# MakiseChris666/MVXNet-Makise

Measured on AMD Instinct MI355X. Metric: KITTI frames/sec (voxelize+VFE+fusion+3Dconv fwd+bwd), higher is better.
Workload: dtype f32 (bf16x6: three bf16 pieces = the f32 operand exactly, six MFMAs per product, f32 accumulate); 1 GPU; S2 ring frames (64-beam model, KITTI-like occupancy), 120000 raw pts -> 20000 pts after crop, grid 10x352x400, T=35, 4 frames/GPU/step: crop+cropToSight+lidar2Img, voxelize, fusion sampling+MLP, VFE, reindex+CML fwd+bwd, all-reduce, AdamW; convmath=bf16x6; mode=hot, frames_per_gpu=4, parallelism=dp1

## Files before the change

mvxnet-makise_amd/csrc/conv3d_split.hip:

```cpp
#include "common.h"
#include "conv_geom.h"
#include "split_common.h"
#include "rowgemm_common.h"

namespace {

constexpr int TH2 = 16;

__global__ void pack_weights_split(const float *__restrict__ w, unsigned short *__restrict__ wsp, int Co, int Ci, int dgrad, int np, int fmt) {
    const int K = dgrad ? Co : Ci, N = dgrad ? Ci : Co;
    const int nch = K / BK;
    const long long total = 27ll * K * N;
    for (long long e = blockIdx.x * (long long)blockDim.x + threadIdx.x; e < total; e += (long long)gridDim.x * blockDim.x) {
        const int k = (int)(e % BK);
        long long r = e / BK;
        const int n = (int)(r % N); r /= N;
        const int ch = (int)(r % nch); r /= nch;
        const int tap = (int)(r % 9);
        const int kd = (int)(r / 9);
        const int a = tap / 3, b = tap % 3;
        const int kk = ch * BK + k;
        const int co = dgrad ? kk : n, ci = dgrad ? n : kk;
        const int kh = dgrad ? 2 - a : a, kw = dgrad ? 2 - b : b;
        float x = w[((((long long)co * Ci + ci) * 3 + kd) * 3 + kh) * 3 + kw];
        const long long row = (((long long)kd * 9 + tap) * nch + ch) * N + n;
        for (int q = 0; q < np; ++q) {
            if (fmt == 0) {
                const __bf16 pb = (__bf16)x;
                wsp[(row * np + q) * BK + k] = __builtin_bit_cast(unsigned short, pb);
                x -= (float)pb;
            } else {
                if (q == 0) x *= SPLIT_F16_WSCALE;
                const _Float16 pb = (_Float16)x;
                wsp[(row * np + q) * BK + k] = __builtin_bit_cast(unsigned short, pb);
                x -= (float)pb;
            }
        }
    }
}

template <int NP, int BKT, int MT, bool WIN, int FMT>
__global__ __launch_bounds__(256, 2) void conv3d_gather_splitT(const float *__restrict__ in,
                                                               const unsigned short *__restrict__ wsp,
                                                               const float *__restrict__ bias,
                                                               float *__restrict__ out, double *__restrict__ stats,
                                                               Geom g, int relu, const int *__restrict__ in_hflag,
                                                               const unsigned char *__restrict__ out_mask,
                                                               const float *__restrict__ bg_pre, int border_active,
                                                               const int *__restrict__ only_tiles,
                                                               unsigned long long *__restrict__ exec_stages,
                                                               const float *__restrict__ in_amax) {
    float a_scale = 1.f;
    if constexpr (FMT == 1) a_scale = split_scale_of(in_amax);
    constexpr int THT = TH * MT, HHT = THT + 2;
    constexpr int ROWBT = NP * BKT * 2 + 16;
    constexpr int HROW = (HW * ROWBT + 255) / 256 * 256;
    constexpr int PPR = NP * BKT / 8;
    constexpr int PT = BN * PPR;
    constexpr int NWU = (3 * PT + 255) / 256;
    constexpr int PARTS = BKT / 4;
    constexpr int NH = (HHT * HW * PARTS + 255) / 256;
    constexpr int KS = BKT / 16;
    __shared__ __attribute__((aligned(256))) unsigned char s_halo[HHT * HROW];
    __shared__ __attribute__((aligned(16))) unsigned char s_w[3][BN * ROWBT];
    __shared__ float s_red[4][2 * BN];
    const int tiles_x = (g.W + TW - 1) / TW, tiles_y8 = (g.H + TH - 1) / TH;
    const int ntiles8 = tiles_x * tiles_y8;
    const int tx = blockIdx.x % tiles_x, tyb = blockIdx.x / tiles_x;
    const int tx0 = tx * TW, ty0 = tyb * THT;
    const int t_top = (MT * tyb) * tiles_x + tx;
    const bool has_bot = MT == 2 && 2 * tyb + 1 < tiles_y8;
    const int t_bot = has_bot ? t_top + tiles_x : t_top;
    const int d = blockIdx.y, nb = blockIdx.z;
    const int tid = threadIdx.x, lane = tid & 63, wv = tid >> 6, li = lane & 31, lh = lane >> 5;
    const int nchunks = g.Cin / BKT;
    if (only_tiles && !(only_tiles[(size_t)d * ntiles8 + t_top] | only_tiles[(size_t)d * ntiles8 + t_bot])) return;
    const bool on_border = tx0 == 0 || ty0 == 0 || tx0 + TW >= g.W || ty0 + THT >= g.H;
    const bool skip_taps = in_hflag && (border_active & 2) && !on_border;
    unsigned skipped = 0;
    int any_flag = 0;
    bool active = true;
    if (in_hflag) {
        for (int kd = 0; kd < 3; ++kd) {
            const int ds = src_depth(g, d, kd);
            if (ds >= 0) {
                const int fl = in_hflag[(size_t)ds * ntiles8 + t_top] | in_hflag[(size_t)ds * ntiles8 + t_bot];
                any_flag |= fl;
                if (skip_taps && !fl) skipped |= 1u << kd;
            }
        }
        active = (((border_active & 1) && on_border) || any_flag) != 0;
    }
    const bool idle_border = in_hflag && (border_active & 2) && on_border && !any_flag;

    f32x16 acc[MT][2];
#pragma unroll
    for (int m = 0; m < MT; ++m)
#pragma unroll
        for (int n = 0; n < 2; ++n)
#pragma unroll
            for (int r = 0; r < 16; ++r) acc[m][n][r] = 0.f;
    int a_base[MT];
#pragma unroll
    for (int m = 0; m < MT; ++m) a_base[m] = (2 * MT * wv + 2 * m + (li >> 4)) * HROW + (li & 15) * ROWBT + lh * 16;
    const int b_base = li * ROWBT + lh * 16;

    typedef unsigned u32x4 __attribute__((ext_vector_type(4)));
    u32x4 wreg[NWU];
    auto load_w3 = [&](int kd, int a, int cc) __attribute__((always_inline)) {
        const int c32 = (cc * BKT) / BK, half = BKT == 16 ? (cc & 1) : 0;
#pragma unroll
        for (int u = 0; u < NWU; ++u) {
            int c = tid + 256 * u;
            if (3 * PT % 256 && c >= 3 * PT) c = 3 * PT - 1;
            const int t = c / PT, rem = c - t * PT;
            const int n = rem / PPR, piece = rem - n * PPR;
            const int q = piece / (BKT / 8), sub = piece - q * (BKT / 8);
            const unsigned char *row = (const unsigned char *)wsp +
                (((((size_t)kd * 9 + a * 3 + t) * (g.Cin / BK) + c32) * g.Cout + (size_t)nb * BN + n) * NP + q) * (BK * 2);
            wreg[u] = *(const u32x4 *)(row + half * 32 + sub * 16);
        }
    };
    auto store_w3 = [&]() __attribute__((always_inline)) {
#pragma unroll
        for (int u = 0; u < NWU; ++u) {
            const int c = tid + 256 * u;
            if (3 * PT % 256 == 0 || c < 3 * PT) {
                const int t = c / PT, rem = c - t * PT;
                const int n = rem / PPR, piece = rem - n * PPR;
                *(u32x4 *)(s_w[t] + n * ROWBT + piece * 16) = wreg[u];
            }
        }
    };

    int kd_l[3] = {0, 0, 0}, ds_l[3] = {0, 0, 0}, nk = 0;
#pragma unroll
    for (int kd = 0; kd < 3; ++kd) {
        const int ds = src_depth(g, d, kd);
        if (ds >= 0 && !((skipped >> kd) & 1u) && !idle_border) {
            if (nk == 0) { kd_l[0] = kd; ds_l[0] = ds; }
            else if (nk == 1) { kd_l[1] = kd; ds_l[1] = ds; }
            else { kd_l[2] = kd; ds_l[2] = ds; }
            ++nk;
        }
    }
    const int nstages = active ? nk * nchunks : 0;
    if (exec_stages && nstages > 0 && threadIdx.x == 0)
        atomicAdd(exec_stages, (unsigned long long)(nk * (g.Cin / BK)) * (has_bot ? 2 : 1));
    auto stage_of = [&](int st, int &kd, int &ds, int &cc) __attribute__((always_inline)) {
        const int i = st / nchunks;
        cc = st - i * nchunks;
        kd = i == 0 ? kd_l[0] : (i == 1 ? kd_l[1] : kd_l[2]);
        ds = i == 0 ? ds_l[0] : (i == 1 ? ds_l[1] : ds_l[2]);
    };
    int h_off[NH], h_lds[NH];
#pragma unroll
    for (int u = 0; u < NH; ++u) {
        const int c = tid + 256 * u;
        h_off[u] = -1;
        h_lds[u] = -1;
        if (c < HHT * HW * PARTS) {
            const int r = c / PARTS, part = c - r * PARTS;
            const int hy = r / HW, hx = r - hy * HW;
            const int gy = ty0 - 1 + hy, gx = tx0 - 1 + hx;
            h_lds[u] = hy * HROW + hx * ROWBT + part * 8;
            if (gy >= 0 && gy < g.H && gx >= 0 && gx < g.W) h_off[u] = (gy * g.W + gx) * g.Cin + part * 4;
        }
    }
    f32x4 hreg[NH];
    auto load_halo = [&](int st) __attribute__((always_inline)) {
        int kd, ds, cc;
        stage_of(st, kd, ds, cc);
        const float *img = in + (size_t)ds * g.H * g.W * g.Cin + cc * BKT;
#pragma unroll
        for (int u = 0; u < NH; ++u)
            hreg[u] = h_off[u] >= 0 ? *(const f32x4 *)(img + h_off[u]) : f32x4{0.f, 0.f, 0.f, 0.f};
    };
    auto store_halo = [&]() __attribute__((always_inline)) {
#pragma unroll
        for (int u = 0; u < NH; ++u)
            if (h_lds[u] >= 0) {
                uint2 pc[NP];
                if constexpr (FMT == 1) hreg[u] *= a_scale;
                split_n<NP, FMT>(hreg[u][0], hreg[u][1], hreg[u][2], hreg[u][3], pc);
#pragma unroll
                for (int q = 0; q < NP; ++q) *(uint2 *)(s_halo + h_lds[u] + q * BKT * 2) = pc[q];
            }
    };
    auto load_wrow = [&](int st, int a) __attribute__((always_inline)) {
        int kd, ds, cc;
        stage_of(st, kd, ds, cc);
        load_w3(kd, a, cc);
    };
    auto compute_row = [&](int a, unsigned colmask) __attribute__((always_inline)) {
#pragma unroll
        for (int b = 0; b < 3; ++b) {
            if (!((colmask >> b) & 1u)) continue;
#pragma unroll
            for (int s2 = 0; s2 < KS; ++s2) {
                bf16x8 b0[NP], b1[NP];
#pragma unroll
                for (int q = 0; q < NP; ++q) {
                    b0[q] = __builtin_bit_cast(bf16x8, *(const uint4 *)(s_w[b] + b_base + q * BKT * 2 + s2 * 32));
                    b1[q] = __builtin_bit_cast(bf16x8, *(const uint4 *)(s_w[b] + b_base + 32 * ROWBT + q * BKT * 2 + s2 * 32));
                }
#pragma unroll
                for (int m = 0; m < MT; ++m) {
                    const int a_off = a_base[m] + a * HROW + b * ROWBT + s2 * 32;
                    bf16x8 av[NP];
#pragma unroll
                    for (int q = 0; q < NP; ++q) av[q] = __builtin_bit_cast(bf16x8, *(const uint4 *)(s_halo + a_off + q * BKT * 2));
                    split_mac2<NP, FMT>(acc[m][0], acc[m][1], av, b0, b1);
                }
            }
        }
    };
    if constexpr (!WIN) {
        if (nstages > 0) {
            load_wrow(0, 0);
            load_halo(0);
        }
        for (int st = 0; st < nstages; ++st) {
            const int nxt = st + 1 < nstages ? st + 1 : st;
            __syncthreads();
            store_halo();
            store_w3();
            __syncthreads();
            load_wrow(st, 1);
            load_halo(nxt);
            compute_row(0, 7u);
            __syncthreads();
            store_w3();
            __syncthreads();
            load_wrow(st, 2);
            compute_row(1, 7u);
            __syncthreads();
            store_w3();
            __syncthreads();
            load_wrow(nxt, 0);
            compute_row(2, 7u);
        }
    } else {
        auto taps_of = [&](int st) __attribute__((always_inline)) -> unsigned {
            unsigned m4 = 0xfu;
            if (g.s2d > 0) m4 = s2d_tap_mask(g.mode == 0 ? ((st % nchunks) * BKT) / g.s2d : (nb * BN) / g.s2d);
            unsigned m9 = 0u;
    #pragma unroll
            for (int a = 0; a < 3; ++a)
    #pragma unroll
                for (int b = 0; b < 3; ++b) {
                    const int ta = g.mode == 0 ? a : 2 - a, tb = g.mode == 0 ? b : 2 - b;
                    const bool in = a >= g.tap_lo && a < g.tap_hi && b >= g.tap_lo && b < g.tap_hi;
                    const bool on = g.s2d > 0 ? ((m4 >> ((ta & 1) * 2 + (tb & 1))) & 1u) && ta < 2 && tb < 2 : true;
                    if (in && on) m9 |= 1u << (a * 3 + b);
                }
            return m9;
        };
        auto first_row = [&](unsigned m9) __attribute__((always_inline)) { return (m9 & 7u) ? 0 : ((m9 & 0x38u) ? 1 : 2); };
        auto next_row = [&](unsigned m9, int a) __attribute__((always_inline)) {
            for (int r = a + 1; r < 3; ++r)
                if ((m9 >> (3 * r)) & 7u) return r;
            return -1;
        };
        int st = 0;
        unsigned m9 = nstages > 0 ? taps_of(0) : 0x1ffu;
        int a = first_row(m9);
        if (nstages > 0) {
            load_wrow(0, a);
            load_halo(0);
        }
        while (st < nstages) {
            const bool first = a == first_row(m9);
            int a2 = next_row(m9, a), st2 = st;
            unsigned m9n = m9;
            if (a2 < 0) {
                st2 = st + 1;
                m9n = st2 < nstages ? taps_of(st2) : m9;
                a2 = first_row(m9n);
            }
            const int stp = st2 < nstages ? st2 : st;
            __syncthreads();
            if (first) store_halo();
            store_w3();
            __syncthreads();
            load_wrow(stp, a2);
            if (first) load_halo(st + 1 < nstages ? st + 1 : st);
            compute_row(a, (m9 >> (3 * a)) & 7u);
            st = st2; a = a2; m9 = m9n;
        }
    }

    if constexpr (FMT == 1) {
        const float o_scale = split_inverse(split_scale_of(in_amax)) * (1.f / SPLIT_F16_WSCALE);
#pragma unroll
        for (int m = 0; m < MT; ++m) { acc[m][0] *= o_scale; acc[m][1] *= o_scale; }
    }
    const int n0 = nb * BN + li, n1 = n0 + 32;
    const float bias0 = bias ? bias[n0] : 0.f, bias1 = bias ? bias[n1] : 0.f;
    float skip0 = 0.f, skip1 = 0.f;
    if (skipped && active) {
        const float *bg_tap = bg_pre + (size_t)g.Dout * g.F * g.Cout + (size_t)d * 3 * g.Cout;
#pragma unroll
        for (int kd = 0; kd < 3; ++kd)
            if ((skipped >> kd) & 1u) { skip0 += bg_tap[kd * g.Cout + n0]; skip1 += bg_tap[kd * g.Cout + n1]; }
    }
    float bgv0 = (bg_pre ? bg_pre[(size_t)d * g.Cout + n0] : 0.f) + bias0, bgv1 = (bg_pre ? bg_pre[(size_t)d * g.Cout + n1] : 0.f) + bias1;
    if (relu) { bgv0 = fmaxf(bgv0, 0.f); bgv1 = fmaxf(bgv1, 0.f); }
    float s1a = 0.f, s2a = 0.f, s1b = 0.f, s2b = 0.f;
#pragma unroll
    for (int m = 0; m < MT; ++m) {
        const int py = ty0 + 2 * MT * wv + 2 * m;
        if (idle_border) {
            const float *bg_cls = bg_pre + (size_t)4 * g.Dout * g.F * g.Cout + (size_t)d * 9 * g.Cout;
#pragma unroll
            for (int r = 0; r < 16; ++r) {
                const int row = mfma32_row(r) + 4 * lh;
                const int gy = py + (row >> 4), gx = tx0 + (row & 15);
                const int q = 3 * (gy == 0 ? 0 : (gy >= g.H - 1 ? 2 : 1)) + (gx == 0 ? 0 : (gx >= g.W - 1 ? 2 : 1));
                acc[m][0][r] = bg_cls[q * g.Cout + n0];
                acc[m][1][r] = bg_cls[q * g.Cout + n1];
            }
        }
        unsigned site_on = active ? 0xffffu : 0u;
        if (out_mask && active) {
            unsigned char mk[16];
#pragma unroll
            for (int r = 0; r < 16; ++r) {
                const int row = mfma32_row(r) + 4 * lh;
                const int gy = min(py + (row >> 4), g.H - 1), gx = min(tx0 + (row & 15), g.W - 1);
                mk[r] = out_mask[((size_t)d * g.H + gy) * g.W + gx];
            }
            site_on = 0u;
#pragma unroll
            for (int r = 0; r < 16; ++r) site_on |= (mk[r] ? 1u : 0u) << r;
        }
#pragma unroll
        for (int r = 0; r < 16; ++r) {
            const int row = mfma32_row(r) + 4 * lh;
            const int gy = py + (row >> 4), gx = tx0 + (row & 15);
            float v0 = (acc[m][0][r] + skip0) + bias0, v1 = (acc[m][1][r] + skip1) + bias1;
            if (relu) { v0 = fmaxf(v0, 0.f); v1 = fmaxf(v1, 0.f); }
            if (out_mask && !((site_on >> r) & 1u)) { v0 = bgv0; v1 = bgv1; }
            if (gy < g.H && gx < g.W) {
                float *o = out + (((size_t)d * g.H + gy) * g.W + gx) * g.Cout;
                o[n0] = v0;
                o[n1] = v1;
                s1a += v0; s2a += v0 * v0;
                s1b += v1; s2b += v1 * v1;
            }
        }
    }
    if (stats) {
        s1a += __shfl_xor(s1a, 32, 64); s2a += __shfl_xor(s2a, 32, 64);
        s1b += __shfl_xor(s1b, 32, 64); s2b += __shfl_xor(s2b, 32, 64);
        __syncthreads();
        if (lh == 0) {
            s_red[wv][li] = s1a; s_red[wv][32 + li] = s1b;
            s_red[wv][BN + li] = s2a; s_red[wv][BN + 32 + li] = s2b;
        }
        __syncthreads();
        if (tid < 2 * BN) {
            const double t = (double)s_red[0][tid] + (double)s_red[1][tid] + (double)s_red[2][tid] + (double)s_red[3][tid];
            const int which = tid / BN, c = tid % BN;
            const unsigned rep = (blockIdx.x + blockIdx.y * gridDim.x) % MVX_REP;
            double *fstats = stats + (size_t)(d / g.Dout) * MVX_REP * 2 * g.Cout;
            atomicAdd(fstats + ((size_t)rep * 2 + which) * g.Cout + nb * BN + c, t);
        }
    }
}

static long long g_split16_min_units = 768;

extern "C" int mvx_tuning_set(int32_t key, int64_t value) {
    if (key == MVX_TUNE_SPLIT16_MIN_UNITS) { g_split16_min_units = value; return MVX_OK; }
    if (key == MVX_TUNE_GATHER_NARROW_MAX_UNITS) { mvxi_gather_narrow_max_units(value); return MVX_OK; }
    if (key == MVX_TUNE_ROWGEMM_K128) { mvxi_rowgemm_k128_enable(value); return MVX_OK; }
    return MVX_EINVAL;
}

static inline int pieces_of(int flags) { return (flags & MVX_FLAG_SPLIT_F16) ? 2 : (flags & MVX_FLAG_SPLIT3) ? 3 : 2; }
static inline int fmt_of(int flags) { return (flags & MVX_FLAG_SPLIT_F16) ? 1 : 0; }

static void launch_gather_split(hipStream_t st, int flags, int planes, int nblocks, const float *in, const unsigned short *wsp,
                                const float *bias, float *out, double *stats, const Geom &g, int relu, const int *in_hflag,
                                const unsigned char *out_mask, const float *bg_pre, int border_active, const int *only_tiles,
                                unsigned long long *exec_stages) {
    const int tiles_x = (int)mvx_cdiv(g.W, TW);
    const long long units16 = (long long)tiles_x * mvx_cdiv(g.H, TH2) * planes * nblocks;
    const bool big = units16 >= g_split16_min_units;
    const dim3 grid(tiles_x * mvx_cdiv(g.H, big ? TH2 : TH), planes, nblocks);
    const bool win = g.tap_lo != 0 || g.tap_hi != 3 || g.s2d > 0;
    const SplitAmax am = mvxi_take_split_amax();
#define MVX_GO(NP_, BK_, MT_, F_)                                                                                                        \
    do {                                                                                                                             \
        if (win)                                                                                                                     \
            hipLaunchKernelGGL((conv3d_gather_splitT<NP_, BK_, MT_, true, F_>), grid, dim3(256), 0, st, in, wsp, bias, out, stats, g,    \
                               relu, in_hflag, out_mask, bg_pre, border_active, only_tiles, exec_stages, am.a);         \
        else                                                                                                                         \
            hipLaunchKernelGGL((conv3d_gather_splitT<NP_, BK_, MT_, false, F_>), grid, dim3(256), 0, st, in, wsp, bias, out, stats, g,   \
                               relu, in_hflag, out_mask, bg_pre, border_active, only_tiles, exec_stages, am.a);         \
    } while (0)
    if (fmt_of(flags)) { if (big) MVX_GO(2, 32, 2, 1); else MVX_GO(2, 32, 1, 1); }
    else if (pieces_of(flags) == 3) { if (big) MVX_GO(3, 16, 2, 0); else MVX_GO(3, 32, 1, 0); }
    else              { if (big) MVX_GO(2, 32, 2, 0); else MVX_GO(2, 32, 1, 0); }
#undef MVX_GO
}

}

extern "C" size_t mvx_conv3d_packed_weight_bytes_split(int32_t cout, int32_t cin, int32_t flags) {
    if (cout <= 0 || cin <= 0) return 0;
    return (size_t)27 * cout * cin * pieces_of(flags) * sizeof(unsigned short);
}

extern "C" int mvx_conv3d_pack_weights_split(const float *w, void *wsplit, int32_t cout, int32_t cin, int32_t for_dgrad,
                                             int32_t flags, void *stream) {
    MVX_CHECK_ARG(w && wsplit && cout > 0 && cin > 0);
    MVX_CHECK_ARG((for_dgrad ? cout : cin) % BK == 0);
    const long long total = 27ll * cout * cin;
    hipLaunchKernelGGL(pack_weights_split, dim3(mvx_cdiv(total, 256) > 2048 ? 2048 : mvx_cdiv(total, 256)), dim3(256), 0,
                       (hipStream_t)stream, w, (unsigned short *)wsplit, cout, cin, for_dgrad, pieces_of(flags), fmt_of(flags));
    MVX_LAUNCH_CHECK();
    return MVX_OK;
}

extern "C" int mvx_conv3d_forward_split(const float *in, const void *wsplit, const float *bias, float *out, double *stats,
                                        int32_t din, int32_t dout, int32_t h, int32_t w, int32_t cin, int32_t cout,
                                        int32_t stride_d, int32_t pad_d, int32_t flags, void *stream) {
    MVX_CHECK_ARG(in && wsplit && out);
    const int relu = flags & MVX_FLAG_RELU;
    int rc = conv_check_forward(din, dout, h, w, cin, cout, stride_d, pad_d);
    if (rc) return rc;
    hipStream_t st = (hipStream_t)stream;
    hipError_t e = conv_zero_stats(stats, nullptr, cout, 1, flags, st);
    if (e != hipSuccess) return (int)e;
    Geom g{din, dout, h, w, cin, cout, stride_d, pad_d, 0};
    launch_gather_split(st, flags, dout, cout / BN, in, (const unsigned short *)wsplit, bias, out, stats, g, relu, nullptr, nullptr, nullptr,
                        0, nullptr, nullptr);
    MVX_LAUNCH_CHECK();
    return MVX_OK;
}

extern "C" int mvx_conv3d_forward_bg_split_frames(const float *in, const void *wsplit, const float *bias, float *out,
                                                  double *stats, int32_t din, int32_t dout, int32_t h, int32_t w, int32_t cin,
                                                  int32_t cout, int32_t stride_d, int32_t pad_d, int32_t flags,
                                                  const int32_t *in_halo_flags, const uint8_t *out_mask, const float *bg_pre,
                                                  int32_t border_active, uint64_t *exec_stages, int32_t n_frames, void *stream) {
    MVX_CHECK_ARG(in && wsplit && out && in_halo_flags && out_mask && bg_pre);
    int rc = conv_check_frames(n_frames);
    if (rc) return rc;
    if ((rc = conv_check_forward(din, dout, h, w, cin, cout, stride_d, pad_d))) return rc;
    hipStream_t st = (hipStream_t)stream;
    hipError_t e = conv_zero_stats(stats, nullptr, cout, n_frames, flags, st);
    if (e != hipSuccess) return (int)e;
    Geom g{din, dout, h, w, cin, cout, stride_d, pad_d, 0, n_frames};
    launch_gather_split(st, flags, dout * n_frames, cout / BN, in, (const unsigned short *)wsplit, bias, out, stats, g,
                        flags & MVX_FLAG_RELU, in_halo_flags, out_mask, bg_pre,
                        (border_active ? 1 : 0) | ((flags & MVX_FLAG_BG_TAPS) ? 2 : 0), nullptr, (unsigned long long *)exec_stages);
    MVX_LAUNCH_CHECK();
    return MVX_OK;
}

extern "C" int mvx_conv3d_forward_bg_split(const float *in, const void *wsplit, const float *bias, float *out, double *stats,
                                           int32_t din, int32_t dout, int32_t h, int32_t w, int32_t cin, int32_t cout,
                                           int32_t stride_d, int32_t pad_d, int32_t flags, const int32_t *in_halo_flags,
                                           const uint8_t *out_mask, const float *bg_pre, int32_t border_active,
                                           void *stream) {
    return mvx_conv3d_forward_bg_split_frames(in, wsplit, bias, out, stats, din, dout, h, w, cin, cout, stride_d, pad_d, flags,
                                              in_halo_flags, out_mask, bg_pre, border_active, nullptr, 1, stream);
}

static int launch_dgrad_split(const float *dz, const void *wsplit_dgrad, float *dx, int32_t din, int32_t dout, int32_t h,
                              int32_t w, int32_t cin, int32_t cout, int32_t stride_d, int32_t pad_d, int32_t flags,
                              const int32_t *only_tiles, uint64_t *exec_stages, int32_t n_frames, void *stream) {
    MVX_CHECK_ARG(dz && wsplit_dgrad && dx);
    int rc = conv_check_frames(n_frames);
    if (rc) return rc;
    if ((rc = conv_check_geom(din, dout, h, w, cout, cin, stride_d, pad_d))) return rc;
    Geom g{dout, din, h, w, cout, cin, stride_d, pad_d, 1, n_frames};
    conv_set_taps2(g, flags, CONV_INPUT_GRAD, BN);
    launch_gather_split((hipStream_t)stream, flags, din * n_frames, cin / BN, dz, (const unsigned short *)wsplit_dgrad, nullptr, dx, nullptr,
                        g, 0, nullptr, nullptr, nullptr, 0, only_tiles, (unsigned long long *)exec_stages);
    MVX_LAUNCH_CHECK();
    return MVX_OK;
}

extern "C" int mvx_conv3d_dgrad_tiles_split_frames(const float *dz, const void *wsplit_dgrad, float *dx, int32_t din,
                                                   int32_t dout, int32_t h, int32_t w, int32_t cin, int32_t cout,
                                                   int32_t stride_d, int32_t pad_d, int32_t flags,
                                                   const int32_t *dx_tile_flags, uint64_t *exec_stages, int32_t n_frames,
                                                   void *stream) {
    MVX_CHECK_ARG(dx_tile_flags);
    return launch_dgrad_split(dz, wsplit_dgrad, dx, din, dout, h, w, cin, cout, stride_d, pad_d, flags, dx_tile_flags,
                              exec_stages, n_frames, stream);
}

extern "C" int mvx_conv3d_dgrad_tiles_split(const float *dz, const void *wsplit_dgrad, float *dx, int32_t din, int32_t dout,
                                            int32_t h, int32_t w, int32_t cin, int32_t cout, int32_t stride_d,
                                            int32_t pad_d, int32_t flags, const int32_t *dx_tile_flags, void *stream) {
    MVX_CHECK_ARG(dx_tile_flags);
    return launch_dgrad_split(dz, wsplit_dgrad, dx, din, dout, h, w, cin, cout, stride_d, pad_d, flags, dx_tile_flags, nullptr, 1,
                              stream);
}

extern "C" int mvx_conv3d_dgrad_split(const float *dz, const void *wsplit_dgrad, float *dx, int32_t din, int32_t dout,
                                      int32_t h, int32_t w, int32_t cin, int32_t cout, int32_t stride_d, int32_t pad_d,
                                      int32_t flags, void *stream) {
    return launch_dgrad_split(dz, wsplit_dgrad, dx, din, dout, h, w, cin, cout, stride_d, pad_d, flags, nullptr, nullptr, 1, stream);
}

extern "C" int mvx_conv2d_forward_split_frames(const float *in, const void *wsplit, const float *bias, float *out, double *stats,
                                               int32_t h, int32_t w, int32_t cin, int32_t cout, int32_t flags,
                                               int32_t n_frames, void *stream) {
    MVX_CHECK_ARG(in && wsplit && out);
    int rc = conv_check_frames(n_frames);
    if (rc) return rc;
    if ((rc = conv_check_geom(1, 1, h, w, cin, cout, 1, 1))) return rc;
    hipStream_t st = (hipStream_t)stream;
    hipError_t e = conv_zero_stats(stats, nullptr, cout, n_frames, flags, st);
    if (e != hipSuccess) return (int)e;
    Geom g{1, 1, h, w, cin, cout, 1, 1, 0, n_frames};
    conv_set_taps2(g, flags, CONV_FORWARD, BK);
    launch_gather_split(st, flags, n_frames, cout / BN, in, (const unsigned short *)wsplit, bias, out, stats, g, flags & MVX_FLAG_RELU,
                        nullptr, nullptr, nullptr, 0, nullptr, nullptr);
    MVX_LAUNCH_CHECK();
    return MVX_OK;
}

extern "C" int mvx_conv2d_dgrad_split_frames(const float *dz, const void *wsplit_dgrad, float *dx, int32_t h, int32_t w,
                                             int32_t cin, int32_t cout, int32_t flags, int32_t n_frames, void *stream) {
    return launch_dgrad_split(dz, wsplit_dgrad, dx, 1, 1, h, w, cin, cout, 1, 1, flags, nullptr, nullptr, n_frames, stream);
}
```

Before: 530.4 frames/s.

## Skip inactive sub-tiles per row-tile in merged MT=2 split conv kernel

Tracks activity and flags separately for each of the MT row-tiles in a block, so a merged two-tile block only loads halo rows and issues MFMAs for the sub-tiles that need computation. It also changes the row mapping so each sub-tile is a contiguous TH-row band, and makes the stats reduction chain in the same order as separate tiles. The aim is to avoid computing empty or background sub-tiles in sparse voxel grids. In exchange it adds masked code paths, more branching, and an extra LDS reduction pass.

```diff
diff --git a/mvxnet-makise_amd/csrc/conv3d_split.hip b/mvxnet-makise_amd/csrc/conv3d_split.hip
--- a/mvxnet-makise_amd/csrc/conv3d_split.hip
+++ b/mvxnet-makise_amd/csrc/conv3d_split.hip
@@ -1,3 +1,4 @@
+#include <type_traits>
 #include "common.h"
 #include "conv_geom.h"
 #include "split_common.h"
@@ -69,29 +70,41 @@
     const int tx = blockIdx.x % tiles_x, tyb = blockIdx.x / tiles_x;
     const int tx0 = tx * TW, ty0 = tyb * THT;
     const int t_top = (MT * tyb) * tiles_x + tx;
-    const bool has_bot = MT == 2 && 2 * tyb + 1 < tiles_y8;
-    const int t_bot = has_bot ? t_top + tiles_x : t_top;
     const int d = blockIdx.y, nb = blockIdx.z;
     const int tid = threadIdx.x, lane = tid & 63, wv = tid >> 6, li = lane & 31, lh = lane >> 5;
     const int nchunks = g.Cin / BKT;
-    if (only_tiles && !(only_tiles[(size_t)d * ntiles8 + t_top] | only_tiles[(size_t)d * ntiles8 + t_bot])) return;
+    constexpr unsigned FULL = (1u << MT) - 1u;
     const bool on_border = tx0 == 0 || ty0 == 0 || tx0 + TW >= g.W || ty0 + THT >= g.H;
-    const bool skip_taps = in_hflag && (border_active & 2) && !on_border;
-    unsigned skipped = 0;
-    int any_flag = 0;
-    bool active = true;
-    if (in_hflag) {
-        for (int kd = 0; kd < 3; ++kd) {
-            const int ds = src_depth(g, d, kd);
-            if (ds >= 0) {
-                const int fl = in_hflag[(size_t)ds * ntiles8 + t_top] | in_hflag[(size_t)ds * ntiles8 + t_bot];
-                any_flag |= fl;
-                if (skip_taps && !fl) skipped |= 1u << kd;
-            }
-        }
-        active = (((border_active & 1) && on_border) || any_flag) != 0;
-    }
-    const bool idle_border = in_hflag && (border_active & 2) && on_border && !any_flag;
+    unsigned valid = 0, flagged = 0, need = 0;
+    int ds_of[3];
+#pragma unroll
+    for (int kd = 0; kd < 3; ++kd) {
+        ds_of[kd] = src_depth(g, d, kd);
+        if (ds_of[kd] >= 0) valid |= 1u << kd;
+    }
+    bool t_on[MT], t_need[MT];
+#pragma unroll
+    for (int m = 0; m < MT; ++m) {
+        const int tr = MT * tyb + m;
+        const bool exists = tr < tiles_y8;
+        const int t = exists ? tr * tiles_x + tx : t_top;
+        t_on[m] = exists && (!only_tiles || only_tiles[(size_t)d * ntiles8 + t] != 0);
+        const bool border = tx == 0 || tx == tiles_x - 1 || tr == 0 || tr >= tiles_y8 - 1;
+        unsigned own = 0;
+        if (in_hflag) {
+#pragma unroll
+            for (int kd = 0; kd < 3; ++kd)
+                if (ds_of[kd] >= 0 && in_hflag[(size_t)ds_of[kd] * ntiles8 + t]) own |= 1u << kd;
+        }
+        flagged |= own;
+        t_need[m] = t_on[m] && (!in_hflag || border || own);
+        if (t_need[m]) need |= 1u << m;
+    }
+    if (only_tiles && !(t_on[0] | t_on[MT - 1])) return;
+    const bool active = !in_hflag || ((border_active & 1) && on_border) || flagged;
+    const bool idle_border = in_hflag && (border_active & 2) && on_border && !flagged;
+    const unsigned skipped = (in_hflag && (border_active & 2) && !on_border) ? valid & ~flagged : 0u;
+    const unsigned run = (active && !idle_border) ? valid & ~skipped : 0u;
 
     f32x16 acc[MT][2];
 #pragma unroll
@@ -102,7 +115,7 @@
             for (int r = 0; r < 16; ++r) acc[m][n][r] = 0.f;
     int a_base[MT];
 #pragma unroll
-    for (int m = 0; m < MT; ++m) a_base[m] = (2 * MT * wv + 2 * m + (li >> 4)) * HROW + (li & 15) * ROWBT + lh * 16;
+    for (int m = 0; m < MT; ++m) a_base[m] = (TH * m + 2 * wv + (li >> 4)) * HROW + (li & 15) * ROWBT + lh * 16;
     const int b_base = li * ROWBT + lh * 16;
 
     typedef unsigned u32x4 __attribute__((ext_vector_type(4)));
@@ -136,22 +149,26 @@
     int kd_l[3] = {0, 0, 0}, ds_l[3] = {0, 0, 0}, nk = 0;
 #pragma unroll
     for (int kd = 0; kd < 3; ++kd) {
-        const int ds = src_depth(g, d, kd);
-        if (ds >= 0 && !((skipped >> kd) & 1u) && !idle_border) {
-            if (nk == 0) { kd_l[0] = kd; ds_l[0] = ds; }
-            else if (nk == 1) { kd_l[1] = kd; ds_l[1] = ds; }
-            else { kd_l[2] = kd; ds_l[2] = ds; }
+        if (((run >> kd) & 1u) && need) {
+            if (nk == 0) { kd_l[0] = kd; ds_l[0] = ds_of[kd]; }
+            else if (nk == 1) { kd_l[1] = kd; ds_l[1] = ds_of[kd]; }
+            else { kd_l[2] = kd; ds_l[2] = ds_of[kd]; }
             ++nk;
         }
     }
-    const int nstages = active ? nk * nchunks : 0;
+    const int nstages = nk * nchunks;
     if (exec_stages && nstages > 0 && threadIdx.x == 0)
-        atomicAdd(exec_stages, (unsigned long long)(nk * (g.Cin / BK)) * (has_bot ? 2 : 1));
+        atomicAdd(exec_stages, (unsigned long long)(nk * (g.Cin / BK) * __builtin_popcount(need)));
     auto stage_of = [&](int st, int &kd, int &ds, int &cc) __attribute__((always_inline)) {
         const int i = st / nchunks;
         cc = st - i * nchunks;
         kd = i == 0 ? kd_l[0] : (i == 1 ? kd_l[1] : kd_l[2]);
         ds = i == 0 ? ds_l[0] : (i == 1 ? ds_l[1] : ds_l[2]);
+    };
+    auto in_rows = [&](int lds, unsigned tm) __attribute__((always_inline)) -> bool {
+        if (tm == FULL) return lds >= 0;
+        const int lo = (tm & 1u) ? 0 : TH * HROW;
+        return (unsigned)(lds - lo) < (unsigned)(HH * HROW);
     };
     int h_off[NH], h_lds[NH];
 #pragma unroll
@@ -168,18 +185,19 @@
         }
     }
     f32x4 hreg[NH];
-    auto load_halo = [&](int st) __attribute__((always_inline)) {
+    auto load_halo = [&](int st, unsigned tm) __attribute__((always_inline)) {
         int kd, ds, cc;
         stage_of(st, kd, ds, cc);
         const float *img = in + (size_t)ds * g.H * g.W * g.Cin + cc * BKT;
 #pragma unroll
         for (int u = 0; u < NH; ++u)
-            hreg[u] = h_off[u] >= 0 ? *(const f32x4 *)(img + h_off[u]) : f32x4{0.f, 0.f, 0.f, 0.f};
-    };
-    auto store_halo = [&]() __attribute__((always_inline)) {
+            hreg[u] = h_off[u] >= 0 && (tm == FULL || in_rows(h_lds[u], tm)) ? *(const f32x4 *)(img + h_off[u])
+                                                                              : f32x4{0.f, 0.f, 0.f, 0.f};
+    };
+    auto store_halo = [&](unsigned tm) __attribute__((always_inline)) {
 #pragma unroll
         for (int u = 0; u < NH; ++u)
-            if (h_lds[u] >= 0) {
+            if (in_rows(h_lds[u], tm)) {
                 uint2 pc[NP];
                 if constexpr (FMT == 1) hreg[u] *= a_scale;
                 split_n<NP, FMT>(hreg[u][0], hreg[u][1], hreg[u][2], hreg[u][3], pc);
@@ -192,7 +210,7 @@
         stage_of(st, kd, ds, cc);
         load_w3(kd, a, cc);
     };
-    auto compute_row = [&](int a, unsigned colmask) __attribute__((always_inline)) {
+    auto compute_row = [&](int a, unsigned colmask, unsigned tm) __attribute__((always_inline)) {
 #pragma unroll
         for (int b = 0; b < 3; ++b) {
             if (!((colmask >> b) & 1u)) continue;
@@ -206,6 +224,7 @@
                 }
 #pragma unroll
                 for (int m = 0; m < MT; ++m) {
+                    if (!((tm >> m) & 1u)) continue;
                     const int a_off = a_base[m] + a * HROW + b * ROWBT + s2 * 32;
                     bf16x8 av[NP];
 #pragma unroll
@@ -215,79 +234,92 @@
             }
         }
     };
-    if constexpr (!WIN) {
-        if (nstages > 0) {
-            load_wrow(0, 0);
-            load_halo(0);
-        }
-        for (int st = 0; st < nstages; ++st) {
-            const int nxt = st + 1 < nstages ? st + 1 : st;
-            __syncthreads();
-            store_halo();
-            store_w3();
-            __syncthreads();
-            load_wrow(st, 1);
-            load_halo(nxt);
-            compute_row(0, 7u);
-            __syncthreads();
-            store_w3();
-            __syncthreads();
-            load_wrow(st, 2);
-            compute_row(1, 7u);
-            __syncthreads();
-            store_w3();
-            __syncthreads();
-            load_wrow(nxt, 0);
-            compute_row(2, 7u);
-        }
+    auto run_stages = [&](auto masked) __attribute__((always_inline)) {
+        auto tiles_of = [&](int st) __attribute__((always_inline)) -> unsigned {
+            if constexpr (decltype(masked)::value) return need;
+            else return FULL;
+        };
+        if constexpr (!WIN) {
+            if (nstages > 0) {
+                load_wrow(0, 0);
+                load_halo(0, tiles_of(0));
+            }
+            for (int st = 0; st < nstages; ++st) {
+                const int nxt = st + 1 < nstages ? st + 1 : st;
+                __syncthreads();
+                store_halo(tiles_of(st));
+                store_w3();
+                __syncthreads();
+                load_wrow(st, 1);
+                load_halo(nxt, tiles_of(nxt));
+                compute_row(0, 7u, tiles_of(st));
+                __syncthreads();
+                store_w3();
+                __syncthreads();
+                load_wrow(st, 2);
+                compute_row(1, 7u, tiles_of(st));
+                __syncthreads();
+                store_w3();
+                __syncthreads();
+                load_wrow(nxt, 0);
+                compute_row(2, 7u, tiles_of(st));
+            }
+        } else {
+            auto taps_of = [&](int st) __attribute__((always_inline)) -> unsigned {
+                unsigned m4 = 0xfu;
+                if (g.s2d > 0) m4 = s2d_tap_mask(g.mode == 0 ? ((st % nchunks) * BKT) / g.s2d : (nb * BN) / g.s2d);
+                unsigned m9 = 0u;
+#pragma unroll
+                for (int a = 0; a < 3; ++a)
+#pragma unroll
+                    for (int b = 0; b < 3; ++b) {
+                        const int ta = g.mode == 0 ? a : 2 - a, tb = g.mode == 0 ? b : 2 - b;
+                        const bool in = a >= g.tap_lo && a < g.tap_hi && b >= g.tap_lo && b < g.tap_hi;
+                        const bool on = g.s2d > 0 ? ((m4 >> ((ta & 1) * 2 + (tb & 1))) & 1u) && ta < 2 && tb < 2 : true;
+                        if (in && on) m9 |= 1u << (a * 3 + b);
+                    }
+                return m9;
+            };
+            auto first_row = [&](unsigned m9) __attribute__((always_inline)) { return (m9 & 7u) ? 0 : ((m9 & 0x38u) ? 1 : 2); };
+            auto next_row = [&](unsigned m9, int a) __attribute__((always_inline)) {
+                for (int r = a + 1; r < 3; ++r)
+                    if ((m9 >> (3 * r)) & 7u) return r;
+                return -1;
+            };
+            int st = 0;
+            unsigned m9 = nstages > 0 ? taps_of(0) : 0x1ffu;
+            int a = first_row(m9);
+            if (nstages > 0) {
+                load_wrow(0, a);
+                load_halo(0, tiles_of(0));
+            }
+            while (st < nstages) {
+                const bool first = a == first_row(m9);
+                int a2 = next_row(m9, a), st2 = st;
+                unsigned m9n = m9;
+                if (a2 < 0) {
+                    st2 = st + 1;
+                    m9n = st2 < nstages ? taps_of(st2) : m9;
+                    a2 = first_row(m9n);
+                }
+                const int stp = st2 < nstages ? st2 : st;
+                __syncthreads();
+                if (first) store_halo(tiles_of(st));
+                store_w3();
+                __syncthreads();
+                load_wrow(stp, a2);
+                const int sth = st + 1 < nstages ? st + 1 : st;
+                if (first) load_halo(sth, tiles_of(sth));
+                compute_row(a, (m9 >> (3 * a)) & 7u, tiles_of(st));
+                st = st2; a = a2; m9 = m9n;
+            }
+        }
+    };
+    if constexpr (MT == 1) {
+        run_stages(std::false_type{});
     } else {
-        auto taps_of = [&](int st) __attribute__((always_inline)) -> unsigned {
-            unsigned m4 = 0xfu;
-            if (g.s2d > 0) m4 = s2d_tap_mask(g.mode == 0 ? ((st % nchunks) * BKT) / g.s2d : (nb * BN) / g.s2d);
-            unsigned m9 = 0u;
-    #pragma unroll
-            for (int a = 0; a < 3; ++a)
-    #pragma unroll
-                for (int b = 0; b < 3; ++b) {
-                    const int ta = g.mode == 0 ? a : 2 - a, tb = g.mode == 0 ? b : 2 - b;
-                    const bool in = a >= g.tap_lo && a < g.tap_hi && b >= g.tap_lo && b < g.tap_hi;
-                    const bool on = g.s2d > 0 ? ((m4 >> ((ta & 1) * 2 + (tb & 1))) & 1u) && ta < 2 && tb < 2 : true;
-                    if (in && on) m9 |= 1u << (a * 3 + b);
-                }
-            return m9;
-        };
-        auto first_row = [&](unsigned m9) __attribute__((always_inline)) { return (m9 & 7u) ? 0 : ((m9 & 0x38u) ? 1 : 2); };
-        auto next_row = [&](unsigned m9, int a) __attribute__((always_inline)) {
-            for (int r = a + 1; r < 3; ++r)
-                if ((m9 >> (3 * r)) & 7u) return r;
-            return -1;
-        };
-        int st = 0;
-        unsigned m9 = nstages > 0 ? taps_of(0) : 0x1ffu;
-        int a = first_row(m9);
-        if (nstages > 0) {
-            load_wrow(0, a);
-            load_halo(0);
-        }
-        while (st < nstages) {
-            const bool first = a == first_row(m9);
-            int a2 = next_row(m9, a), st2 = st;
-            unsigned m9n = m9;
-            if (a2 < 0) {
-                st2 = st + 1;
-                m9n = st2 < nstages ? taps_of(st2) : m9;
-                a2 = first_row(m9n);
-            }
-            const int stp = st2 < nstages ? st2 : st;
-            __syncthreads();
-            if (first) store_halo();
-            store_w3();
-            __syncthreads();
-            load_wrow(stp, a2);
-            if (first) load_halo(st + 1 < nstages ? st + 1 : st);
-            compute_row(a, (m9 >> (3 * a)) & 7u);
-            st = st2; a = a2; m9 = m9n;
-        }
+        if (need == FULL) run_stages(std::false_type{});
+        else run_stages(std::true_type{});
     }
 
     if constexpr (FMT == 1) {
@@ -297,6 +329,8 @@
     }
     const int n0 = nb * BN + li, n1 = n0 + 32;
     const float bias0 = bias ? bias[n0] : 0.f, bias1 = bias ? bias[n1] : 0.f;
+    float bgv0 = (bg_pre ? bg_pre[(size_t)d * g.Cout + n0] : 0.f) + bias0, bgv1 = (bg_pre ? bg_pre[(size_t)d * g.Cout + n1] : 0.f) + bias1;
+    if (relu) { bgv0 = fmaxf(bgv0, 0.f); bgv1 = fmaxf(bgv1, 0.f); }
     float skip0 = 0.f, skip1 = 0.f;
     if (skipped && active) {
         const float *bg_tap = bg_pre + (size_t)g.Dout * g.F * g.Cout + (size_t)d * 3 * g.Cout;
@@ -304,12 +338,14 @@
         for (int kd = 0; kd < 3; ++kd)
             if ((skipped >> kd) & 1u) { skip0 += bg_tap[kd * g.Cout + n0]; skip1 += bg_tap[kd * g.Cout + n1]; }
     }
-    float bgv0 = (bg_pre ? bg_pre[(size_t)d * g.Cout + n0] : 0.f) + bias0, bgv1 = (bg_pre ? bg_pre[(size_t)d * g.Cout + n1] : 0.f) + bias1;
-    if (relu) { bgv0 = fmaxf(bgv0, 0.f); bgv1 = fmaxf(bgv1, 0.f); }
     float s1a = 0.f, s2a = 0.f, s1b = 0.f, s2b = 0.f;
+    unsigned in_image[MT];
 #pragma unroll
     for (int m = 0; m < MT; ++m) {
-        const int py = ty0 + 2 * MT * wv + 2 * m;
+        in_image[m] = 0u;
+        if (!t_on[m]) continue;
+        const int py = ty0 + TH * m + 2 * wv;
+        const bool computed = active && t_need[m];
         if (idle_border) {
             const float *bg_cls = bg_pre + (size_t)4 * g.Dout * g.F * g.Cout + (size_t)d * 9 * g.Cout;
 #pragma unroll
@@ -321,8 +357,8 @@
                 acc[m][1][r] = bg_cls[q * g.Cout + n1];
             }
         }
-        unsigned site_on = active ? 0xffffu : 0u;
-        if (out_mask && active) {
+        unsigned site_on = computed ? 0xffffu : 0u;
+        if (out_mask && computed) {
             unsigned char mk[16];
 #pragma unroll
             for (int r = 0; r < 16; ++r) {
@@ -345,16 +381,70 @@
                 float *o = out + (((size_t)d * g.H + gy) * g.W + gx) * g.Cout;
                 o[n0] = v0;
                 o[n1] = v1;
-                s1a += v0; s2a += v0 * v0;
-                s1b += v1; s2b += v1 * v1;
+                if constexpr (MT == 1) {
+                    s1a += v0; s2a += v0 * v0;
+                    s1b += v1; s2b += v1 * v1;
+                } else {
+                    in_image[m] |= 1u << r;
+                    acc[m][0][r] = v0;
+                    acc[m][1][r] = v1;
+                }
             }
         }
     }
     if (stats) {
-        s1a += __shfl_xor(s1a, 32, 64); s2a += __shfl_xor(s2a, 32, 64);
-        s1b += __shfl_xor(s1b, 32, 64); s2b += __shfl_xor(s2b, 32, 64);
-        __syncthreads();
-        if (lh == 0) {
+        int red_row = wv;
+        if constexpr (MT == 2) {
+            float *hand = (float *)s_halo;
+            float ch[MT][4];
+            __syncthreads();
+            auto chain = [&](int m) __attribute__((always_inline)) {
+#pragma unroll
+                for (int r = 0; r < 16; ++r)
+                    if ((in_image[m] >> r) & 1u) {
+                        const float v0 = acc[m][0][r], v1 = acc[m][1][r];
+                        ch[m][0] += v0; ch[m][1] += v0 * v0;
+                        ch[m][2] += v1; ch[m][3] += v1 * v1;
+                    }
+            };
+            if (!(wv & 1)) {
+#pragma unroll
+                for (int m = 0; m < MT; ++m) {
+#pragma unroll
+                    for (int k = 0; k < 4; ++k) ch[m][k] = 0.f;
+                    chain(m);
+#pragma unroll
+                    for (int k = 0; k < 4; ++k) hand[(((wv >> 1) * MT + m) * 4 + k) * 64 + lane] = ch[m][k];
+                }
+            }
+            __syncthreads();
+            if (wv & 1) {
+#pragma unroll
+                for (int m = 0; m < MT; ++m) {
+#pragma unroll
+                    for (int k = 0; k < 4; ++k) ch[m][k] = hand[(((wv >> 1) * MT + m) * 4 + k) * 64 + lane];
+                    chain(m);
+                }
+            }
+#pragma unroll
+            for (int m = 0; m < MT; ++m)
+#pragma unroll
+                for (int k = 0; k < 4; ++k) ch[m][k] += __shfl_xor(ch[m][k], 32, 64);
+            if ((wv & 1) && lh == 0) {
+#pragma unroll
+                for (int m = 0; m < MT; ++m) {
+                    const int j = 2 * m + (wv >> 1);
+                    s_red[j][li] = ch[m][0]; s_red[j][32 + li] = ch[m][2];
+                    s_red[j][BN + li] = ch[m][1]; s_red[j][BN + 32 + li] = ch[m][3];
+                }
+            }
+            red_row = -1;
+        } else {
+            s1a += __shfl_xor(s1a, 32, 64); s2a += __shfl_xor(s2a, 32, 64);
+            s1b += __shfl_xor(s1b, 32, 64); s2b += __shfl_xor(s2b, 32, 64);
+            __syncthreads();
+        }
+        if (red_row >= 0 && lh == 0) {
             s_red[wv][li] = s1a; s_red[wv][32 + li] = s1b;
             s_red[wv][BN + li] = s2a; s_red[wv][BN + 32 + li] = s2b;
         }
```

New measurement: 534.8 frames/s (median of 6 runs). No clear change (+0.8%).
